# MAGIC-AI4Med/KEEP

Measured on AMD Instinct MI355X. Metric: 224x224 tiles encoded/sec (whole node), higher is better.
Workload: dtype fp16+mxfp4

## Files before the change

### keep_amd/csrc/common.h

```cpp
#pragma once
#include <hip/hip_runtime.h>
#include <stdint.h>

typedef _Float16 f16;
typedef _Float16 f16x2 __attribute__((ext_vector_type(2)));
typedef _Float16 f16x4 __attribute__((ext_vector_type(4)));
typedef _Float16 f16x8 __attribute__((ext_vector_type(8)));
typedef float f32x4 __attribute__((ext_vector_type(4)));
typedef float f32x16 __attribute__((ext_vector_type(16)));

#define KEEP_WAVE 64

__device__ __forceinline__ void split_f16(float x, f16& hi, f16& lo) {
    asm("" : "+v"(x));
    hi = (f16)x;
    lo = (f16)(x - (float)hi);
}

__device__ __forceinline__ unsigned char clip8_fixed(int v) {
    v >>= 22;
    return (unsigned char)(v < 0 ? 0 : (v > 255 ? 255 : v));
}
__device__ __forceinline__ float gelu_erf(float x) {
    return 0.5f * x * (1.0f + erff(x * 0.70710678118654752440f));
}

__device__ __forceinline__ float wave_sum(float v) {
#pragma unroll
    for (int o = 32; o > 0; o >>= 1) v += __shfl_xor(v, o);
    return v;
}
__device__ __forceinline__ float wave_max(float v) {
#pragma unroll
    for (int o = 32; o > 0; o >>= 1) v = fmaxf(v, __shfl_xor(v, o));
    return v;
}

__host__ __device__ __forceinline__ int64_t blk_off(int m, int k, int KT) {
    return ((int64_t)(m >> 8) * KT + (k >> 5)) * 8192 + ((m & 255) << 5) + (k & 31);
}
static inline size_t blk_elems(int64_t M, int64_t K) { return (size_t)((M + 255) / 256 * 256) * (size_t)K; }


struct KeepTune {
    int gemm_impl = 0;
    int gemm_skinny_m = 320;
    int skinny_wide = 1;
    int gemm_splitk_tiles = 64;
    int sgemv_m = 16;
    int ln_impl = 2;
    int attn_waves = 16;
    int gemm_persistent = 1;
    int gemm_ablate = 0;
    long long* dbg = nullptr;
};

enum GemmEpi : int {
    EPI_F16      = 0,
    EPI_GELU_F16 = 1,
    EPI_RESID_LS = 2,
    EPI_PATCH    = 3,
    EPI_RESID_F32= 4,
    EPI_PARTIAL  = 5,
    EPI_TOP2     = 6,
};

struct GemmParams {
    const f16* a_hi; const f16* a_lo;
    const f16* w_hi; const f16* w_lo;
    int M, N, K;
    int nseg;
    int comp;
    const unsigned char* a_q; const unsigned char* a_sc;
    const unsigned char* w_q; const unsigned char* w_sc;
    unsigned char* out_q; unsigned char* out_sc;
    const float* bias;
    const float* ls;
    const float* pos;
    float* resid;
    float* out_f32;
    f16* out_hi; f16* out_lo;
    int out_kt;
    int patches_per_img;
    const float* ln_gamma; const float* ln_beta; float ln_eps;
    f16* ln_out_hi; f16* ln_out_lo; float* ln_out_f32;
    int top2_c; float* top2_partial; int top2_kpad;
    int impl_hint;
    int ksplit;
    float* splitk_ws; size_t splitk_bytes;
    long long* dbg;
    int ablate;
    const KeepTune* tune;
};

int launch_gemm_f16(const GemmParams& p, int epi, hipStream_t s);
constexpr int GEMM_DID_LN = 1;
constexpr int SKINNY_MAX_M = 1024;
constexpr size_t SKINNY_WS_BYTES = (size_t)448 * 256 * 256 * 4;
int launch_gemm_splitk_reduce(const GemmParams& p, int epi, const float* ws, int S, hipStream_t s);
int launch_gemm_f16_skinny(const GemmParams& p, int epi, float* ws, size_t ws_bytes, hipStream_t s);

struct AttnParams {
    const f16* qkv_hi; const f16* qkv_lo;
    f16* out_hi; f16* out_lo;
    int out_kt;
    const int64_t* mask;
    int batch, ntok, heads;
    int q_rows;
    int split;
    f16* cls_hi; f16* cls_lo;
    float* part_ws; size_t part_bytes;
    int key0, kcount;
    float* part_out; const float* part_in;
    float scale;
    long long* dbg;
    const KeepTune* tune;
};
int launch_attention(const AttnParams& p, hipStream_t s);
int launch_attention_long(const AttnParams& p, hipStream_t s);
constexpr int ATT_PART_FLOATS = 66;
int launch_attention_cls_probs(const f16* qkv_hi, const f16* qkv_lo, int batch, int ntok, int heads, float scale, float* out, hipStream_t s);
constexpr int ROLLOUT_MAX_TOKENS = 272;
int launch_attention_rollout_step(const f16* qkv_hi, const f16* qkv_lo, int batch, int ntok, int heads, float scale, float residual,
                                  const float* r_in, float* r_out, int q_rows, float* a_tmp, hipStream_t s);

struct LnParams {
    const float* x; int64_t x_stride;
    const float* add;
    const float* gamma; const float* beta;
    int rows, D; float eps;
    f16* out_hi; f16* out_lo;
    int out_kt;
    float* out_f32; int64_t out_f32_stride;
    unsigned char* out_q; unsigned char* out_sc;
    int out_q_hi_only;
    const KeepTune* tune;
};
int launch_layernorm(const LnParams& p, hipStream_t s);

enum SgemmAct : int { ACT_NONE = 0, ACT_GELU = 1, ACT_TANH = 2 };
struct SgemmParams {
    const float* a; int64_t lda;
    const float* b; int64_t ldb;
    float* out; int64_t ldo;
    const float* bias;
    int M, N, K;
    float scale; int act;
    const KeepTune* tune;
};
int launch_sgemm_f32(const SgemmParams& p, hipStream_t s);

__device__ __forceinline__ int block_exclusive_scan256(int v, int* s, int* total) {
    const int t = threadIdx.x;
    s[t] = v;
    __syncthreads();
    for (int o = 1; o < 256; o <<= 1) {
        const int a = t >= o ? s[t - o] : 0;
        __syncthreads();
        s[t] += a;
        __syncthreads();
    }
    const int incl = s[t];
    *total = s[255];
    __syncthreads();
    return incl - v;
}

void launch_region_grid(const unsigned char* region, int64_t row_stride, int ps, int gx, int64_t ncells, int patch, int step, int sat_min,
                        int min_pixels, unsigned char* keep, int* counts, int* offsets, int32_t* cell_xy, int64_t* n_out, hipStream_t s);
void launch_region_check_cells(const int32_t* cell_xy, int B, int64_t H, int64_t W, int patch, int* bad, hipStream_t s);
void launch_region_patches_u8(const unsigned char* region, int64_t row_stride, int ps, const int32_t* cell_xy, int B, int patch,
                              const int* xb, const int* xk, int xks, const int* yb, const int* yk, int yks, unsigned char* tmp,
                              unsigned char* out, hipStream_t s);
void launch_region_compact(const unsigned char* keep, int gx, int64_t ncells, int step, int* counts, int* offsets, int32_t* cell_xy,
                           int64_t* n_out, hipStream_t s);
constexpr int REGION_MAX_PATCH = 32768;
constexpr int REGION_GRID_CHUNK = 2048;

constexpr int64_t TISSUE_MAX_PIXELS = (int64_t)1 << 30;
int launch_tissue_median_hist(const unsigned char* thumb, int64_t row_stride, int ps, int h, int w, int ksize, unsigned char* med, int* hist,
                              hipStream_t s);
void launch_tissue_mask(const unsigned char* med, int h, int w, int thr, int close, int min_hole, int min_area, unsigned char* tmp, int* labels,
                        int* info, int* err, unsigned char* mask, hipStream_t s);
void launch_tissue_grid_cells(const unsigned char* mask, int64_t mh, int64_t mw, int64_t ds, int gx, int64_t ncells, int patch, int step,
                              int64_t ox, int64_t oy, int mode, unsigned char* keep, hipStream_t s);

void launch_cc_label(const unsigned char* img, int h, int w, int conn8, int* labels, int* info, int* err, hipStream_t s);

constexpr int REGIONS_COLS = 14;
constexpr int REGIONS_SCAN_CHUNK = 2048;
void launch_regions_label(const unsigned char* mask, int h, int w, int conn8, int min_area, int* roots, int* info, int* counts, int* offsets,
                          int* err, int* labels_out, int64_t* n_out, hipStream_t s);
void launch_regions_table(const int* labels, int h, int w, int64_t n, const int64_t* acc, int64_t* table, hipStream_t s);

constexpr int64_t OUTLINE_MAX_PIXELS = (int64_t)1 << 28;
constexpr int OUTLINE_COLS = 8;
constexpr int OUTLINE_CHUNK = 2048;
constexpr int OUTLINE_FLAG_WORDS = 96;
constexpr int OUTLINE_MAX_WIDTH = 16;
size_t outline_count_workspace_bytes(int64_t npix);
// ... 114 lines not shown
```

### keep_amd/csrc/engine.hip

```cpp
#include "handle.h"
#include "quant4.h"

#include <algorithm>
#include <cmath>
#include <cstring>

namespace {

constexpr int64_t TXT_GRAPH_ROWS = 4096;

const char* kTagNames[T_COUNT] = {
    "vit.im2col", "vit.patch", "vit.ln", "vit.qkv", "vit.attn", "vit.proj", "vit.fc1", "vit.fc2", "vit.head",
    "text.embed", "text.ln", "text.qkv", "text.attn", "text.out", "text.ffn1", "text.ffn2", "text.pool", "sim",
    "vit.qkv.x", "vit.attn.x", "vit.proj.x", "vit.fc1.x", "vit.fc2.x", "vit.tail"};

struct Scope {
    keep_handle* h; int tag; hipStream_t s;
    Scope(keep_handle* h_, int t, hipStream_t s_) : h(h_), tag(t), s(s_) { h->prof_begin(tag, s); }
    ~Scope() { h->prof_end(tag, s); }
};

size_t align_up(size_t x, size_t a = 256) { return (x + a - 1) / a * a; }

struct Carver {
// ... 501 lines not shown

struct RollArgs { int start; float residual; float* out; char* scratch; int64_t scratch_bytes; };
struct RollPlan { size_t buf, lane, total; };
RollPlan rollout_scratch(int64_t B, int ntok, const VitPlan& plan) {
    RollPlan r{};
    const int64_t live = std::min<int64_t>(B, plan.per * plan.lanes);
    r.buf = align_up((size_t)plan.per * ntok * ntok * sizeof(float));
    r.lane = 3 * r.buf;
    r.total = r.lane * (size_t)((live + plan.per - 1) / plan.per);
    return r;
}
int encode_image_run(keep_handle* h, const void* pixels, int pix_dtype, int64_t B, float* out, hipStream_t s, int gh = 14, int gw = 14,
                     int tap_block = -1, float* tap_out = nullptr, const RollArgs* roll = nullptr) {
    const int ntok = gh * gw + 1;
    const bool g14 = gh == 14 && gw == 14;
    const float* pos = nullptr;
    int rc = vit_pos_table(h, gh, gw, &pos);
    if (rc) return rc;
    const size_t px = pix_dtype == KEEP_PIX_F32 ? 4 : (pix_dtype == KEEP_PIX_U8_HWC ? 1 : 2);
    const size_t tile_vals = (size_t)3 * (gh * 16) * (gw * 16);
    const bool graph = h->use_graphs && !h->prof_mode && B * ntok <= SKINNY_MAX_M && B <= h->max_tiles && !tap_out && !roll;
    const VitPlan plan = vit_plan(h, B, ntok, tile_vals * px, graph);
    const RollPlan rp = roll ? rollout_scratch(B, ntok, plan) : RollPlan{};
    if (roll && (int64_t)rp.total > roll->scratch_bytes)
        return h->fail(KEEP_EINVAL, "rollout scratch of %lld bytes, %lld needed (keep_rollout_scratch_bytes)", (long long)roll->scratch_bytes, (long long)rp.total);
    rc = ensure_arena(h, plan.total);
    if (rc) return rc;
    if (graph) {
        const size_t ob = (size_t)B * h->proj_dim * sizeof(float);
        char* st_pix = h->arena + plan.o_pix;
        float* st_out = (float*)(h->arena + plan.o_out);
        HIPCHK(h, hipMemcpyAsync(st_pix, pixels, (size_t)B * tile_vals * px, hipMemcpyDeviceToDevice, s));
        char key[96];
        if (g14) snprintf(key, sizeof key, "img|%lld|%d|%d", (long long)B, pix_dtype, h->precision);
        else snprintf(key, sizeof key, "img|%lld|%d|%d|%dx%d", (long long)B, pix_dtype, h->precision, gh, gw);
        rc = graph_run(h, key, s, [&](hipStream_t cs) {
            VitLane L{};
            L.Bc = (int)B; L.pixels = st_pix; L.pix_dtype = pix_dtype; L.out = st_out; L.s = cs;
            L.gh = gh; L.gw = gw; L.ntok = ntok; L.pos = pos;
            L.ws = carve_vit(h, h->arena, L.Bc, plan.split, ntok);
            int r = vit_begin(h, L);
            for (int i = 0; !r && i < h->vit_depth; ++i) r = vit_layer(h, L, i);
            return r ? r : vit_end(h, L);
        });
        if (rc) return rc;
        HIPCHK(h, hipMemcpyAsync(out, st_out, ob, hipMemcpyDeviceToDevice, s));
        return KEEP_OK;
    }
    const int lanes = plan.lanes;
    const int64_t per = plan.per;
    if (lanes > 1) {
        if (!h->ev_fork) HIPCHK(h, hipEventCreateWithFlags(&h->ev_fork, hipEventDisableTiming));
        for (int l = 0; l < lanes; ++l) {
            if (!h->aux[l]) HIPCHK(h, hipStreamCreateWithFlags(&h->aux[l], hipStreamNonBlocking));
            if (!h->ev_join[l]) HIPCHK(h, hipEventCreateWithFlags(&h->ev_join[l], hipEventDisableTiming));
        }
        HIPCHK(h, hipEventRecord(h->ev_fork, s));
        for (int l = 0; l < lanes; ++l) HIPCHK(h, hipStreamWaitEvent(h->aux[l], h->ev_fork, 0));
    }
    for (int64_t b0 = 0; b0 < B; b0 += per * lanes) {
        VitLane L[4];
        int nl = 0;
        for (int l = 0; l < lanes; ++l) {
            const int64_t lo = b0 + l * per;
            if (lo >= B) break;
            VitLane& x = L[nl++];
            x.Bc = (int)((B - lo) < per ? (B - lo) : per);
            x.pixels = (const char*)pixels + (size_t)lo * tile_vals * px;
            x.pix_dtype = pix_dtype;
            x.out = out + lo * h->proj_dim;
            x.s = lanes > 1 ? h->aux[l] : s;
            x.gh = gh; x.gw = gw; x.ntok = ntok; x.pos = pos;
            if (tap_out) { x.tap_block = tap_block; x.tap_out = tap_out + lo * h->vit_heads * ntok; }
            if (roll) {
                float* base = (float*)(roll->scratch + (size_t)l * rp.lane);
                x.roll_start = roll->start; x.roll_res = roll->residual; x.roll_out = roll->out + lo * ntok;
                x.roll_r[0] = base; x.roll_r[1] = base + rp.buf / sizeof(float); x.roll_a = base + 2 * (rp.buf / sizeof(float));
            }
            x.ws = carve_vit(h, h->arena + (size_t)l * plan.lane_bytes, x.Bc, plan.split, ntok);
        }
        for (int l = 0; l < nl; ++l) if ((rc = vit_begin(h, L[l]))) return rc;
        for (int i = 0; i < h->vit_depth; ++i)
            for (int l = 0; l < nl; ++l) if ((rc = vit_layer(h, L[l], i))) return rc;
        for (int l = 0; l < nl; ++l) if ((rc = vit_end(h, L[l]))) return rc;
    }
    if (lanes > 1)
        for (int l = 0; l < lanes; ++l) {
            HIPCHK(h, hipEventRecord(h->ev_join[l], h->aux[l]));
            HIPCHK(h, hipStreamWaitEvent(s, h->ev_join[l], 0));
        }
    return KEEP_OK;
}


int similarity_run(keep_handle* h, const float* img, const float* txt, int64_t N, int64_t P, int64_t D, float scale, int mode,
                   void* out, int32_t* argmax_out, hipStream_t s) {
    Scope sc(h, T_SIM, s);
    if (h->tune.sgemv_m > 0 && launch_sim_small(img, txt, (int)N, (int)P, (int)D, scale, mode, out, argmax_out, s) == 0)
        return check_launch(h, "similarity");
    if (h->tune.sgemv_m > 0 && launch_sim_mid(img, txt, (int)N, (int)P, (int)D, scale, mode, out, argmax_out, s) == 0)
        return check_launch(h, "similarity");
    float* logits = (float*)out;
    const bool need_tmp = (mode == KEEP_SIM_ARGMAX && !out) || mode == KEEP_SIM_SOFTMAX_F16 || mode == KEEP_SIM_TOP2SCORE;
    const int nb = (int)((N + 255) / 256);
    if (need_tmp) {
        const size_t bytes = align_up((size_t)N * P * 4) + align_up((size_t)nb * 4) + 256;
        int rc = ensure_arena(h, bytes);
        if (rc) return rc;
        logits = (float*)h->arena;
    }
    SgemmParams g{};
    g.tune = &h->tune;
    g.a = img; g.lda = D; g.b = txt; g.ldb = D; g.out = logits; g.ldo = P; g.bias = nullptr;
    g.M = (int)N; g.N = (int)P; g.K = (int)D; g.act = ACT_NONE;
    g.scale = (mode == KEEP_SIM_RAW || mode == KEEP_SIM_ARGMAX) ? scale : 1.0f;
    if (launch_sgemm_f32(g, s)) return h->fail(KEEP_EUNSUPPORTED, "similarity shape");
    if (mode == KEEP_SIM_ARGMAX) launch_row_argmax(logits, (int)N, (int)P, argmax_out, s);
    else if (mode == KEEP_SIM_SOFTMAX) launch_row_softmax(logits, (int)N, (int)P, scale, logits, s);
    else if (mode == KEEP_SIM_SOFTMAX_F16) launch_row_softmax_f16(logits, (int)N, (int)P, scale, (f16*)out, s);
    else if (mode == KEEP_SIM_TOP2SCORE) {
        float* partial = (float*)(h->arena + align_up((size_t)N * P * 4));
        launch_top2_score(logits, (int)N, (int)P, partial, (float*)out, s);
    }
    return check_launch(h, "similarity");
}


enum : unsigned { OPT_REPLAN = 1,
                  OPT_WRITEONLY = 2 };
struct Opt { const char* name; int keep_handle::* hm; int KeepTune::* tm; bool is_bool; int lo, hi; const char* msg; unsigned flags; };
constexpr int NO_MAX = 0x7fffffff;
static_assert(SKINNY_MAX_M == 1024, "the gemm_skinny_m message below spells the bound out");
const Opt kOptions[] = {
    {"graphs", &keep_handle::use_graphs, nullptr, true, 0, 0, nullptr, 0},
    {"strict_blocks", &keep_handle::strict_blocks, nullptr, false, 0, NO_MAX, "strict_blocks < 0", 0},
    {"comp_full_blocks", &keep_handle::comp_full_blocks, nullptr, false, 0, NO_MAX, "comp_full_blocks < 0", OPT_REPLAN},
    {"comp_mlp_blocks", &keep_handle::comp_mlp_blocks, nullptr, false, 0, NO_MAX, "comp_mlp_blocks < 0", OPT_REPLAN},
    {"comp_qkv", &keep_handle::comp_qkv, nullptr, true, 0, 0, nullptr, OPT_REPLAN},
    {"comp_qkv_from", &keep_handle::comp_qkv_from, nullptr, false, 0, NO_MAX, "comp_qkv_from < 0", OPT_REPLAN},
    {"comp_min_tiles", &keep_handle::comp_min_tiles, nullptr, false, 24, NO_MAX, "comp_min_tiles must be >= 24 (the compensated product needs the 256x256 kernel)", 0},
    {"fused_screening", &keep_handle::fused_screening, nullptr, false, 0, 2, "fused_screening must be 0..2", OPT_WRITEONLY},
    {"max_tiles", &keep_handle::max_tiles, nullptr, false, 1, NO_MAX, "max_tiles < 1", 0},
    {"max_prompts", &keep_handle::max_prompts, nullptr, false, 1, NO_MAX, "max_prompts < 1", 0},
    {"cls_tail", &keep_handle::cls_tail, nullptr, true, 0, 0, nullptr, 0},
    {"patch_split", &keep_handle::patch_split, nullptr, true, 0, 0, nullptr, 0},
    {"grid_plan", &keep_handle::grid_plan, nullptr, false, 0, 2, "grid_plan must be 0, 1 or 2", 0},
    {"bias_correction", &keep_handle::bias_correction, nullptr, true, 0, 0, nullptr, 0},
    {"streams", &keep_handle::n_streams, nullptr, false, 1, 4, "streams must be 1..4", 0},
    {"lane_min_tiles", &keep_handle::lane_min_tiles, nullptr, false, 6, NO_MAX, "lane_min_tiles must be >= 6", OPT_WRITEONLY},
    {"gemm_persistent", nullptr, &KeepTune::gemm_persistent, false, 0, 1024, "gemm_persistent must be 0..1024", 0},
    {"gemm_splitk_tiles", nullptr, &KeepTune::gemm_splitk_tiles, false, 0, 256, "gemm_splitk_tiles must be 0..256", 0},
    {"sgemv_m", nullptr, &KeepTune::sgemv_m, false, 0, 16, "sgemv_m must be 0..16", 0},
    {"skinny_wide", nullptr, &KeepTune::skinny_wide, true, 0, 0, nullptr, 0},
    {"gemm_skinny_m", nullptr, &KeepTune::gemm_skinny_m, false, 0, SKINNY_MAX_M, "gemm_skinny_m must be 0..1024", 0},
    {"ln_impl", nullptr, &KeepTune::ln_impl, false, 0, 2, "ln_impl must be 0, 1 or 2", 0},
};
const Opt* find_opt(const char* name) {
    for (const Opt& o : kOptions) if (!strcmp(name, o.name)) return &o;
    return nullptr;
}
int& opt_value(keep_handle* h, const Opt& o) { return o.hm ? h->*o.hm : h->tune.*o.tm; }

}

extern "C" {

const char* keep_version(void) { return "keep_hip 0.1 (gfx950)"; }

int keep_create(int device_id, keep_handle** out) {
    if (!out) return KEEP_EINVAL;
    *out = nullptr;
    int n = 0;
    if (hipGetDeviceCount(&n) != hipSuccess || device_id < 0 || device_id >= n) return KEEP_EHIP;
    DevGuard guard(device_id);
    if (!guard.ok) return KEEP_EHIP;
    keep_handle* h = new keep_handle();
    h->device = device_id;
    if (hipMalloc(&h->err_flag, 4 * sizeof(int)) != hipSuccess) { delete h; return KEEP_ENOMEM; }
    hipMemset(h->err_flag, 0, 4 * sizeof(int));
    *out = h;
    return KEEP_OK;
}

int keep_destroy(keep_handle* h) {
    if (!h) return KEEP_OK;
    DevGuard guard(h->device);
    hipDeviceSynchronize();
    h->prof_collect();
    for (auto& e : h->pool) { hipEventDestroy(e.first); hipEventDestroy(e.second); }
    for (auto& kv : h->w) { if (kv.second.f32) hipFree(kv.second.f32); if (kv.second.hi) hipFree(kv.second.hi); if (kv.second.lo) hipFree(kv.second.lo);
                            if (kv.second.q) hipFree(kv.second.q); if (kv.second.sc) hipFree(kv.second.sc); }
    if (h->tune.dbg) hipFree(h->tune.dbg);
    for (float* v : h->owned_vecs) hipFree(v);
    h->free_cal();
    h->drop_pos_cache();
    for (auto& l : h->blayers) { if (l.qkv.hi) hipFree(l.qkv.hi); if (l.qkv.lo) hipFree(l.qkv.lo); if (l.qkv_b) hipFree(l.qkv_b); }
    drop_graphs(h);
    if (h->cap_stream) hipStreamDestroy(h->cap_stream);
    if (h->arena) hipFree(h->arena);
    if (h->cls_buf) hipFree(h->cls_buf);
    if (h->err_flag) hipFree(h->err_flag);
    for (int l = 0; l < 4; ++l) { if (h->aux[l]) hipStreamDestroy(h->aux[l]); if (h->ev_join[l]) hipEventDestroy(h->ev_join[l]); }
    if (h->ev_fork) hipEventDestroy(h->ev_fork);
    delete h;
    return KEEP_OK;
}

const char* keep_last_error(keep_handle* h) { return h ? h->err.c_str() : "null handle"; }

int keep_set_option(keep_handle* h, const char* name, double value) {
    if (!h || !name) return KEEP_EINVAL;
    const std::string n(name);
    const int v = (int)value;
    ++h->opt_epoch;
    KeepTune& t = h->tune;
    if (const Opt* o = find_opt(name)) {
        if (!o->is_bool && (v < o->lo || v > o->hi)) return h->fail(KEEP_EINVAL, "%s", o->msg);
        opt_value(h, *o) = o->is_bool ? (v ? 1 : 0) : v;
        if (o->flags & OPT_REPLAN) h->plan_from_prefix();
        if (o->hm == &keep_handle::cls_tail && h->bias_ready && h->cal_cls_tail != h->cls_tail) h->bias_ready = false;
    }
    else if (n == "label_margin") { if (!(value >= 0.0) || value > 2.0) return h->fail(KEEP_EINVAL, "label_margin must be in [0, 2]"); h->label_margin = (float)value; }
    else if (n == "precision") { if (v != KEEP_PREC_FP16 && v != KEEP_PREC_STRICT && v != KEEP_PREC_COMP) return h->fail(KEEP_EINVAL, "precision %d", v); h->precision = v; }
    else if (n == "proj_impl") { if (v != 0 && v != 2128) return h->fail(KEEP_EINVAL, "proj_impl must be 0 or 2128"); h->proj_impl = v; }
    else if (n == "attn_waves") { if (v != 4 && v != 8 && v != 16) return h->fail(KEEP_EINVAL, "attn_waves must be 4, 8 or 16 (16: persistent double-buffered kernel for the image tower)"); t.attn_waves = v; }
    else if (n == "gemm_impl") { if (v != 0 && v != 128 && v != 256) return h->fail(KEEP_EINVAL, "gemm_impl %d (0, 128, 256)", v); t.gemm_impl = v; }
#ifdef KEEP_DIAGNOSTICS
    else if (n == "gemm_ablate") { t.gemm_ablate = v; }
    else if (n == "gemm_dbg") {
        if (v && !t.dbg) { HIPCHK(h, hipMalloc(&t.dbg, (size_t)65536 * 4 * sizeof(long long))); HIPCHK(h, hipMemset(t.dbg, 0, (size_t)65536 * 4 * sizeof(long long))); }
        if (!v && t.dbg) { hipFree(t.dbg); t.dbg = nullptr; }
    }
#endif
    else return h->fail(KEEP_EINVAL, "unknown option %s", name);
    return KEEP_OK;
}
double keep_get_option(keep_handle* h, const char* name) {
    if (!h || !name) return -1;
    const std::string n(name);
    if (const Opt* o = find_opt(name)) return (o->flags & OPT_WRITEONLY) ? -1 : opt_value(h, *o);
    if (n == "label_margin") return h->label_margin;
    if (n == "precision") return h->precision;
    if (n == "proj_impl") return h->proj_impl;
    if (n == "attn_waves") return h->tune.attn_waves;
    if (n == "gemm_impl") return h->tune.gemm_impl;
    if (n == "plan_custom") return h->plan_custom ? 1 : 0;
    if (n == "bias_ready") return h->bias_ready ? 1 : 0;
    if (n == "graph_count") return (double)h->graphs.size();
    return -1;
}

int keep_set_block_precision(keep_handle* h, int block, int attn_mode, int mlp_mode) {
    if (!h) return KEEP_EINVAL;
    if (block < 0 || block >= keep_handle::MAX_BLOCKS) return h->fail(KEEP_EINVAL, "block %d outside 0..%d", block, keep_handle::MAX_BLOCKS - 1);
    if (attn_mode > KEEP_ATTN_COMPQKV_PROJ_CLS || mlp_mode > KEEP_MLP_CLS) return h->fail(KEEP_EINVAL, "attn_mode %d (0..5) / mlp_mode %d (0..4); negative = leave", attn_mode, mlp_mode);
    ++h->opt_epoch;
    if (attn_mode >= 0) h->attn_mode[block] = (unsigned char)attn_mode;
    if (mlp_mode >= 0) h->mlp_mode[block] = (unsigned char)mlp_mode;
    h->plan_custom = true;
    return KEEP_OK;
}
int keep_get_block_precision(keep_handle* h, int block, int* attn_mode, int* mlp_mode) {
    if (!h) return KEEP_EINVAL;
    if (block < 0 || block >= keep_handle::MAX_BLOCKS) return h->fail(KEEP_EINVAL, "block %d outside 0..%d", block, keep_handle::MAX_BLOCKS - 1);
    if (attn_mode) *attn_mode = h->attn_mode[block];
    if (mlp_mode) *mlp_mode = h->mlp_mode[block];
    return KEEP_OK;
}

int keep_reserve(keep_handle* h, int64_t tiles, int64_t prompts, int64_t seq) {
    if (!h || !h->finalized) return h ? h->fail(KEEP_ESTATE, "weights not finalised") : KEEP_EINVAL;
    KEEP_ON_DEVICE(h);
    size_t need = 0;
    if (tiles > 0 && h->vit_depth) need = vit_plan(h, tiles, 197, (size_t)3 * 224 * 224 * 4, tiles * 197 <= SKINNY_MAX_M).total;
    if (prompts > 0 && seq > 0 && h->bert_layers) need = std::max(need, txt_plan(h, prompts, seq, prompts * seq <= TXT_GRAPH_ROWS).total);
    return ensure_arena(h, need);
}
int64_t keep_workspace_bytes(keep_handle* h) { return h ? (int64_t)h->arena_bytes : 0; }

int keep_encode_image(keep_handle* h, const void* pixels, int pix_dtype, int64_t B, float* out, void* stream) {
    if (!h) return KEEP_EINVAL;
    if (!h->finalized || !h->vit_depth) return h->fail(KEEP_ESTATE, "image tower not loaded / finalised");
    if (!pixels || !out || B < 0) return h->fail(KEEP_EINVAL, "null pointer or negative batch");
    if (pix_dtype < KEEP_PIX_F32 || pix_dtype > KEEP_PIX_U8_HWC) return h->fail(KEEP_EINVAL, "pixel dtype %d", pix_dtype);
    if (B == 0) return KEEP_OK;
    KEEP_ON_DEVICE(h);
    return encode_image_run(h, pixels, pix_dtype, B, out, (hipStream_t)stream);
}

int keep_encode_image_hw(keep_handle* h, const void* pixels, int pix_dtype, int64_t B, int64_t H, int64_t W, float* out, void* stream) {
    if (!h) return KEEP_EINVAL;
    if (!h->finalized || !h->vit_depth) return h->fail(KEEP_ESTATE, "image tower not loaded / finalised");
    if (!pixels || !out || B < 0) return h->fail(KEEP_EINVAL, "null pointer or negative batch");
    if (pix_dtype < KEEP_PIX_F32 || pix_dtype > KEEP_PIX_U8_HWC) return h->fail(KEEP_EINVAL, "pixel dtype %d", pix_dtype);
    if (H < 16 || W < 16 || H % 16 || W % 16) return h->fail(KEEP_EINVAL, "image size %lldx%lld: H and W must be positive multiples of 16", (long long)H, (long long)W);
    const int64_t gh = H / 16, gw = W / 16;
    if (gh * gw + 1 > 65536) return h->fail(KEEP_EUNSUPPORTED, "image size %lldx%lld: more than 65536 patches", (long long)H, (long long)W);
    if (B == 0) return KEEP_OK;
    KEEP_ON_DEVICE(h);
    const int prec = h->precision;
    if (!(gh == 14 && gw == 14) && !h->grid_keeps_plan((int)(gh * gw + 1)) && prec == KEEP_PREC_COMP) h->precision = KEEP_PREC_STRICT;
    const int rc = encode_image_run(h, pixels, pix_dtype, B, out, (hipStream_t)stream, (int)gh, (int)gw);
    h->precision = prec;
    return rc;
}

// ... 451 lines not shown
```

### keep_amd/csrc/gemm_f16_skinny.hip

```cpp
#include "gemm_epilogue.h"

namespace keepk {

constexpr int SK_BM = 32, SK_BN = 128;

__global__ __launch_bounds__(256)
void gemm_skinny_partial_kernel(GemmParams p, float* __restrict__ part, int steps_per_split) {
    const int lane = threadIdx.x & 63, wave = threadIdx.x >> 6;
    const int n0 = blockIdx.x * SK_BN + wave * 32, m0 = blockIdx.y * SK_BM, split = blockIdx.z;
    const int KT = p.K / 32;
    const int kt0 = split * steps_per_split;
    const int kt1 = min(KT, kt0 + steps_per_split);
    const int r = lane & 31, half = lane >> 5;
    const int m = m0 + r, n = n0 + r;
    const int64_t a_base = (int64_t)(m >> 8) * KT * 8192 + ((m & 255) << 5) + half * 8;
    const int64_t w_base = (int64_t)(n >> 8) * KT * 8192 + ((n & 255) << 5) + half * 8;
    f32x16 acc;
#pragma unroll
    for (int i = 0; i < 16; ++i) acc[i] = 0.f;
    for (int seg = 0; seg < p.nseg; ++seg) {
        const f16* A = (seg == 1 ? p.a_lo : p.a_hi) + a_base;
        const f16* W = (seg == 2 ? p.w_lo : p.w_hi) + w_base;
        int kt = kt0;
        for (; kt + 2 <= kt1; kt += 2) {
            const f16x8 a0 = *reinterpret_cast<const f16x8*>(A + (int64_t)kt * 8192);
            const f16x8 w0 = *reinterpret_cast<const f16x8*>(W + (int64_t)kt * 8192);
            const f16x8 a1 = *reinterpret_cast<const f16x8*>(A + (int64_t)kt * 8192 + 16);
            const f16x8 w1 = *reinterpret_cast<const f16x8*>(W + (int64_t)kt * 8192 + 16);
            const f16x8 a2 = *reinterpret_cast<const f16x8*>(A + (int64_t)(kt + 1) * 8192);
            const f16x8 w2 = *reinterpret_cast<const f16x8*>(W + (int64_t)(kt + 1) * 8192);
            const f16x8 a3 = *reinterpret_cast<const f16x8*>(A + (int64_t)(kt + 1) * 8192 + 16);
            const f16x8 w3 = *reinterpret_cast<const f16x8*>(W + (int64_t)(kt + 1) * 8192 + 16);
            acc = __builtin_amdgcn_mfma_f32_32x32x16_f16(w0, a0, acc, 0, 0, 0);
            acc = __builtin_amdgcn_mfma_f32_32x32x16_f16(w1, a1, acc, 0, 0, 0);
            acc = __builtin_amdgcn_mfma_f32_32x32x16_f16(w2, a2, acc, 0, 0, 0);
            acc = __builtin_amdgcn_mfma_f32_32x32x16_f16(w3, a3, acc, 0, 0, 0);
        }
        for (; kt < kt1; ++kt) {
            const f16x8 a0 = *reinterpret_cast<const f16x8*>(A + (int64_t)kt * 8192);
            const f16x8 w0 = *reinterpret_cast<const f16x8*>(W + (int64_t)kt * 8192);
            const f16x8 a1 = *reinterpret_cast<const f16x8*>(A + (int64_t)kt * 8192 + 16);
            const f16x8 w1 = *reinterpret_cast<const f16x8*>(W + (int64_t)kt * 8192 + 16);
            acc = __builtin_amdgcn_mfma_f32_32x32x16_f16(w0, a0, acc, 0, 0, 0);
            acc = __builtin_amdgcn_mfma_f32_32x32x16_f16(w1, a1, acc, 0, 0, 0);
        }
    }
    if (m < p.M) {
        float* o = part + ((int64_t)split * p.M + m) * p.N + n0 + half * 4;
#pragma unroll
        for (int rg = 0; rg < 4; ++rg) {
            f32x4 v;
#pragma unroll
            for (int e = 0; e < 4; ++e) v[e] = acc[rg * 4 + e];
            *reinterpret_cast<f32x4*>(o + rg * 8) = v;
        }
    }
}

constexpr int SK2_BM = 128, SK2_BN = 128;

__global__ __launch_bounds__(256)
void gemm_skinny_partial_wide_kernel(GemmParams p, float* __restrict__ part, int steps_per_split) {
    const int lane = threadIdx.x & 63, wave = threadIdx.x >> 6;
    const int wm = wave >> 1, wn = wave & 1;
    const int n0 = blockIdx.x * SK2_BN + wn * 64, m0 = blockIdx.y * SK2_BM + wm * 64, split = blockIdx.z;
    const int KT = p.K / 32;
    const int kt0 = split * steps_per_split;
    const int kt1 = min(KT, kt0 + steps_per_split);
    const int r = lane & 31, half = lane >> 5;
    int64_t a_base[2], w_base[2];
#pragma unroll
    for (int f = 0; f < 2; ++f) {
        const int m = m0 + f * 32 + r, n = n0 + f * 32 + r;
        a_base[f] = (int64_t)(m >> 8) * KT * 8192 + ((m & 255) << 5) + half * 8;
        w_base[f] = (int64_t)(n >> 8) * KT * 8192 + ((n & 255) << 5) + half * 8;
    }
    f32x16 acc[2][2];
#pragma unroll
    for (int i = 0; i < 2; ++i)
#pragma unroll
        for (int j = 0; j < 2; ++j)
#pragma unroll
            for (int e = 0; e < 16; ++e) acc[i][j][e] = 0.f;
    const int nk = kt1 - kt0, steps = nk > 0 ? nk * p.nseg : 0;
    auto frag = [&](int st, f16x8 (&a)[2][2], f16x8 (&w)[2][2]) {
        const int seg = st / nk, kt = kt0 + (st - seg * nk);
        const f16* A = seg == 1 ? p.a_lo : p.a_hi;
        const f16* W = seg == 2 ? p.w_lo : p.w_hi;
#pragma unroll
        for (int f = 0; f < 2; ++f)
#pragma unroll
            for (int k = 0; k < 2; ++k) {
                a[f][k] = *reinterpret_cast<const f16x8*>(A + a_base[f] + (int64_t)kt * 8192 + k * 16);
                w[f][k] = *reinterpret_cast<const f16x8*>(W + w_base[f] + (int64_t)kt * 8192 + k * 16);
            }
    };
    auto fma8 = [&](const f16x8 (&a)[2][2], const f16x8 (&w)[2][2]) {
#pragma unroll
        for (int k = 0; k < 2; ++k)
#pragma unroll
            for (int i = 0; i < 2; ++i)
#pragma unroll
                for (int j = 0; j < 2; ++j) acc[i][j] = __builtin_amdgcn_mfma_f32_32x32x16_f16(w[j][k], a[i][k], acc[i][j], 0, 0, 0);
    };
    f16x8 a0[2][2], w0[2][2], a1[2][2], w1[2][2];
    if (steps > 0) frag(0, a0, w0);
    int st = 0;
    for (; st + 2 <= steps; st += 2) {
        frag(st + 1, a1, w1);
        fma8(a0, w0);
        if (st + 2 < steps) frag(st + 2, a0, w0);
        fma8(a1, w1);
    }
    if (st < steps) fma8(a0, w0);
#pragma unroll
    for (int i = 0; i < 2; ++i) {
        const int m = m0 + i * 32 + r;
        if (m >= p.M) continue;
#pragma unroll
        for (int j = 0; j < 2; ++j) {
            float* o = part + ((int64_t)split * p.M + m) * p.N + n0 + j * 32 + half * 4;
#pragma unroll
            for (int rg = 0; rg < 4; ++rg) {
                f32x4 v;
#pragma unroll
                for (int e = 0; e < 4; ++e) v[e] = acc[i][j][rg * 4 + e];
                *reinterpret_cast<f32x4*>(o + rg * 8) = v;
            }
        }
    }
}

template <int EPI>
__global__ __launch_bounds__(256)
void gemm_skinny_reduce_kernel(GemmParams p, const float* __restrict__ part, int S) {
    const int64_t idx = (int64_t)blockIdx.x * 256 + threadIdx.x;
    const int nq = p.N / 4;
    if (idx >= (int64_t)p.M * nq) return;
    const int m = (int)(idx / nq), n = (int)(idx - (int64_t)m * nq) * 4;
    f32x4 v = *reinterpret_cast<const f32x4*>(part + (int64_t)m * p.N + n);
    for (int s = 1; s < S; ++s) {
        const f32x4 x = *reinterpret_cast<const f32x4*>(part + ((int64_t)s * p.M + m) * p.N + n);
#pragma unroll
        for (int e = 0; e < 4; ++e) v[e] += x[e];
    }
    const f32x4 bias = *reinterpret_cast<const f32x4*>(p.bias + n);
#pragma unroll
    for (int e = 0; e < 4; ++e) v[e] += bias[e];
    int prow; int64_t orow;
    gemm_epilogue_row<EPI>(p, m, prow, orow);
    const int64_t o = orow * p.N + n;
    if (EPI == EPI_F16 || EPI == EPI_GELU_F16) {
        if (EPI == EPI_GELU_F16) {
            f32x2 a = {v[0], v[1]}, b = {v[2], v[3]};
            if (p.out_lo) { a = gelu_fast2(a); b = gelu_fast2(b); }
            else { a = gelu_fast2_fp16(a); b = gelu_fast2_fp16(b); }
            v[0] = a[0]; v[1] = a[1]; v[2] = b[0]; v[3] = b[1];
        }
        f16x4 h, l;
#pragma unroll
        for (int e = 0; e < 4; ++e) { f16 hh, ll; split_f16(v[e], hh, ll); h[e] = hh; l[e] = ll; }
        const int64_t oo = p.out_kt > 0 ? blk_off((int)orow, n, p.out_kt) : o;
        *reinterpret_cast<f16x4*>(p.out_hi + oo) = h;
        if (p.out_lo) *reinterpret_cast<f16x4*>(p.out_lo + oo) = l;
    } else if (EPI == EPI_RESID_LS) {
        const f32x4 g = *reinterpret_cast<const f32x4*>(p.ls + n);
        f32x4 r = *reinterpret_cast<const f32x4*>(p.resid + o);
#pragma unroll
        for (int e = 0; e < 4; ++e) r[e] += __fmul_rn(g[e], v[e]);
        *reinterpret_cast<f32x4*>(p.resid + o) = r;
    } else if (EPI == EPI_PATCH) {
        const f32x4 pe = *reinterpret_cast<const f32x4*>(p.pos + (int64_t)prow * p.N + n);
#pragma unroll
        for (int e = 0; e < 4; ++e) v[e] += pe[e];
        *reinterpret_cast<f32x4*>(p.resid + o) = v;
    } else {
        const f32x4 r = *reinterpret_cast<const f32x4*>(p.resid + o);
#pragma unroll
        for (int e = 0; e < 4; ++e) v[e] += r[e];
        *reinterpret_cast<f32x4*>(p.out_f32 + o) = v;
    }
}

template <int EPI>
__global__ __launch_bounds__(256)
void gemm_skinny_reduce_ln_kernel(GemmParams p, const float* __restrict__ part, int S) {
    __shared__ float red[2][4];
    const int m = blockIdx.x, t = threadIdx.x, n = t * 4;
    const bool on = n < p.N;
    f32x4 r = {0.f, 0.f, 0.f, 0.f};
    if (on) {
        f32x4 v = *reinterpret_cast<const f32x4*>(part + (int64_t)m * p.N + n);
        for (int s = 1; s < S; ++s) {
            const f32x4 x = *reinterpret_cast<const f32x4*>(part + ((int64_t)s * p.M + m) * p.N + n);
#pragma unroll
            for (int e = 0; e < 4; ++e) v[e] += x[e];
        }
        const f32x4 bias = *reinterpret_cast<const f32x4*>(p.bias + n);
        const int64_t o = (int64_t)m * p.N + n;
        r = *reinterpret_cast<const f32x4*>(p.resid + o);
        if (EPI == EPI_RESID_LS) {
            const f32x4 g = *reinterpret_cast<const f32x4*>(p.ls + n);
#pragma unroll
            for (int e = 0; e < 4; ++e) r[e] += __fmul_rn(g[e], v[e] + bias[e]);
            *reinterpret_cast<f32x4*>(p.resid + o) = r;
        } else {
#pragma unroll
            for (int e = 0; e < 4; ++e) r[e] = (v[e] + bias[e]) + r[e];
            if (p.ln_out_f32 != p.out_f32) *reinterpret_cast<f32x4*>(p.out_f32 + o) = r;
        }
    }
    const int wave = t >> 6, lane = t & 63;
    float sum = wave_sum(r[0] + r[1] + r[2] + r[3]);
    if (lane == 0) red[0][wave] = sum;
    __syncthreads();
    const float mean = (red[0][0] + red[0][1] + red[0][2] + red[0][3]) / (float)p.N;
    float sq = 0.f;
    if (on) {
#pragma unroll
        for (int e = 0; e < 4; ++e) { r[e] -= mean; sq += r[e] * r[e]; }
    }
    sq = wave_sum(sq);
    if (lane == 0) red[1][wave] = sq;
    __syncthreads();
    const float rstd = 1.0f / sqrtf((red[1][0] + red[1][1] + red[1][2] + red[1][3]) / (float)p.N + p.ln_eps);
    if (!on) return;
    const f32x4 g = *reinterpret_cast<const f32x4*>(p.ln_gamma + n);
    const f32x4 bt = *reinterpret_cast<const f32x4*>(p.ln_beta + n);
    f32x4 y; f16x4 h, l;
#pragma unroll
    for (int e = 0; e < 4; ++e) {
        y[e] = r[e] * rstd * g[e] + bt[e];
        f16 hh, ll; split_f16(y[e], hh, ll); h[e] = hh; l[e] = ll;
    }
    if (p.ln_out_f32) *reinterpret_cast<f32x4*>(p.ln_out_f32 + (int64_t)m * p.N + n) = y;
    const int64_t oo = blk_off(m, n, p.N / 32);
    *reinterpret_cast<f16x4*>(p.ln_out_hi + oo) = h;
    if (p.ln_out_lo) *reinterpret_cast<f16x4*>(p.ln_out_lo + oo) = l;
}

}
using namespace keepk;

bool skinny_wide(int M, const KeepTune* t = nullptr) { return M >= 64 && (!t || t->skinny_wide); }

int skinny_splits(int M, int N, int K, const KeepTune* t = nullptr) {
    const bool wide = skinny_wide(M, t);
    const int tiles = wide ? ((M + SK2_BM - 1) / SK2_BM) * (N / SK2_BN) : ((M + SK_BM - 1) / SK_BM) * (N / SK_BN), ks = K / 32;
    int S = ((wide ? 256 : 768) + tiles - 1) / tiles;
    if (S > ks / 2) S = ks / 2;
    if (S > 16) S = 16;
    return S < 1 ? 1 : S;
}

size_t skinny_ws_bytes(int M, int N, int K) { return (size_t)skinny_splits(M, N, K) * M * N * sizeof(float); }

int launch_gemm_f16_skinny(const GemmParams& p, int epi, float* ws, size_t ws_bytes, hipStream_t s) {
    if (!ws || p.N % SK_BN || p.K % 32 || p.M < 1) return -1;
    const int S = skinny_splits(p.M, p.N, p.K, p.tune);
    if ((size_t)S * p.M * p.N * sizeof(float) > ws_bytes) return -1;
    const int KT = p.K / 32, per = (KT + S - 1) / S;
    dim3 block(256);
    if (skinny_wide(p.M, p.tune)) hipLaunchKernelGGL(gemm_skinny_partial_wide_kernel, dim3(p.N / SK2_BN, (p.M + SK2_BM - 1) / SK2_BM, S), block, 0, s, p, ws, per);
    else hipLaunchKernelGGL(gemm_skinny_partial_kernel, dim3(p.N / SK_BN, (p.M + SK_BM - 1) / SK_BM, S), block, 0, s, p, ws, per);
    return launch_gemm_splitk_reduce(p, epi, ws, S, s);
}

int launch_gemm_splitk_reduce(const GemmParams& p, int epi, const float* ws, int S, hipStream_t s) {
    dim3 block(256);
    if (p.ln_gamma && p.ln_out_hi && (epi == EPI_RESID_LS || epi == EPI_RESID_F32) && p.N <= 1024) {
        if (epi == EPI_RESID_LS) hipLaunchKernelGGL(gemm_skinny_reduce_ln_kernel<EPI_RESID_LS>, dim3(p.M), block, 0, s, p, ws, S);
        else hipLaunchKernelGGL(gemm_skinny_reduce_ln_kernel<EPI_RESID_F32>, dim3(p.M), block, 0, s, p, ws, S);
        return GEMM_DID_LN;
    }
    const int64_t items = (int64_t)p.M * (p.N / 4);
    dim3 rg((unsigned)((items + 255) / 256));
    switch (epi) {
        case EPI_F16:       hipLaunchKernelGGL(gemm_skinny_reduce_kernel<EPI_F16>, rg, block, 0, s, p, ws, S); break;
        case EPI_GELU_F16:  hipLaunchKernelGGL(gemm_skinny_reduce_kernel<EPI_GELU_F16>, rg, block, 0, s, p, ws, S); break;
        case EPI_RESID_LS:  hipLaunchKernelGGL(gemm_skinny_reduce_kernel<EPI_RESID_LS>, rg, block, 0, s, p, ws, S); break;
        case EPI_PATCH:     hipLaunchKernelGGL(gemm_skinny_reduce_kernel<EPI_PATCH>, rg, block, 0, s, p, ws, S); break;
        default:            hipLaunchKernelGGL(gemm_skinny_reduce_kernel<EPI_RESID_F32>, rg, block, 0, s, p, ws, S); break;
    }
    return 0;
}
```

Before: 7043.

## Add fused three-segment skinny wide GEMM kernel with register ring prefetch

Adds a split-K skinny wide kernel for compensated (hi/lo, nseg==3) products that handles all three product segments in one pass over K. It loads A and W hi/lo slices together and keeps separate main and correction accumulators. The older kernel loops over segments and re-streams the operands three times. A DEPTH-slot register ring prefetches upcoming K slices to hide global-load latency. The cost is much higher register pressure (two 4x4 accumulator sets plus four slices of four planes), which may reduce occupancy or cause spills.

```diff
diff --git a/keep_amd/csrc/common.h b/keep_amd/csrc/common.h
--- a/keep_amd/csrc/common.h
+++ b/keep_amd/csrc/common.h
@@ -46,6 +46,7 @@
     int gemm_impl = 0;
     int gemm_skinny_m = 320;
     int skinny_wide = 1;
+    int skinny_fused = 1;
     int gemm_splitk_tiles = 64;
     int sgemv_m = 16;
     int ln_impl = 2;
diff --git a/keep_amd/csrc/engine.hip b/keep_amd/csrc/engine.hip
--- a/keep_amd/csrc/engine.hip
+++ b/keep_amd/csrc/engine.hip
@@ -677,6 +677,7 @@
     {"gemm_splitk_tiles", nullptr, &KeepTune::gemm_splitk_tiles, false, 0, 256, "gemm_splitk_tiles must be 0..256", 0},
     {"sgemv_m", nullptr, &KeepTune::sgemv_m, false, 0, 16, "sgemv_m must be 0..16", 0},
     {"skinny_wide", nullptr, &KeepTune::skinny_wide, true, 0, 0, nullptr, 0},
+    {"skinny_fused", nullptr, &KeepTune::skinny_fused, true, 0, 0, nullptr, 0},
     {"gemm_skinny_m", nullptr, &KeepTune::gemm_skinny_m, false, 0, SKINNY_MAX_M, "gemm_skinny_m must be 0..1024", 0},
     {"ln_impl", nullptr, &KeepTune::ln_impl, false, 0, 2, "ln_impl must be 0, 1 or 2", 0},
 };
diff --git a/keep_amd/csrc/gemm_f16_skinny.hip b/keep_amd/csrc/gemm_f16_skinny.hip
--- a/keep_amd/csrc/gemm_f16_skinny.hip
+++ b/keep_amd/csrc/gemm_f16_skinny.hip
@@ -131,6 +131,101 @@
     }
 }
 
+#ifndef SK2_FUSED_DEPTH
+#define SK2_FUSED_DEPTH 4
+#endif
+
+struct Sk2Slice { f16x8 ah[4], al[4], wh[4], wl[4]; };
+struct Sk2Planes { const f16* ah; const f16* al; const f16* wh; const f16* wl; int64_t a[4], w[4]; };
+
+__device__ __forceinline__ void sk2_load(Sk2Slice& s, const Sk2Planes& q, int kt) {
+#pragma unroll
+    for (int f = 0; f < 4; ++f) {
+        const int64_t ao = q.a[f] + (int64_t)kt * 8192, wo = q.w[f] + (int64_t)kt * 8192;
+        s.ah[f] = *reinterpret_cast<const f16x8*>(q.ah + ao);
+        s.al[f] = *reinterpret_cast<const f16x8*>(q.al + ao);
+        s.wh[f] = *reinterpret_cast<const f16x8*>(q.wh + wo);
+        s.wl[f] = *reinterpret_cast<const f16x8*>(q.wl + wo);
+    }
+}
+
+__device__ __forceinline__ void sk2_fma48(const Sk2Slice& s, f32x4 (&main)[4][4], f32x4 (&corr)[4][4]) {
+#pragma unroll
+    for (int i = 0; i < 4; ++i)
+#pragma unroll
+        for (int j = 0; j < 4; ++j) main[i][j] = __builtin_amdgcn_mfma_f32_16x16x32_f16(s.wh[j], s.ah[i], main[i][j], 0, 0, 0);
+#pragma unroll
+    for (int i = 0; i < 4; ++i)
+#pragma unroll
+        for (int j = 0; j < 4; ++j) corr[i][j] = __builtin_amdgcn_mfma_f32_16x16x32_f16(s.wh[j], s.al[i], corr[i][j], 0, 0, 0);
+#pragma unroll
+    for (int i = 0; i < 4; ++i)
+#pragma unroll
+        for (int j = 0; j < 4; ++j) corr[i][j] = __builtin_amdgcn_mfma_f32_16x16x32_f16(s.wl[j], s.ah[i], corr[i][j], 0, 0, 0);
+}
+
+template <int DEPTH>
+__global__ __launch_bounds__(256)
+void gemm_skinny_partial_wide_fused_kernel(GemmParams p, float* __restrict__ part, int steps_per_split) {
+    const int lane = threadIdx.x & 63, wave = threadIdx.x >> 6;
+    const int wm = wave >> 1, wn = wave & 1;
+    const int n0 = blockIdx.x * SK2_BN + wn * 64, m0 = blockIdx.y * SK2_BM + wm * 64, split = blockIdx.z;
+    const int KT = p.K / 32;
+    const int kt0 = split * steps_per_split;
+    const int kt1 = min(KT, kt0 + steps_per_split);
+    const int r = lane & 15, quarter = lane >> 4;
+    Sk2Planes q{p.a_hi, p.a_lo, p.w_hi, p.w_lo, {0, 0, 0, 0}, {0, 0, 0, 0}};
+#pragma unroll
+    for (int f = 0; f < 4; ++f) {
+        const int m = m0 + f * 16 + r, n = n0 + f * 16 + r;
+        q.a[f] = (int64_t)(m >> 8) * KT * 8192 + ((m & 255) << 5) + quarter * 8;
+        q.w[f] = (int64_t)(n >> 8) * KT * 8192 + ((n & 255) << 5) + quarter * 8;
+    }
+    f32x4 main[4][4], corr[4][4];
+#pragma unroll
+    for (int i = 0; i < 4; ++i)
+#pragma unroll
+        for (int j = 0; j < 4; ++j)
+#pragma unroll
+            for (int e = 0; e < 4; ++e) main[i][j][e] = corr[i][j][e] = 0.f;
+    Sk2Slice ring[DEPTH];
+    const int nk = kt1 - kt0 > 0 ? kt1 - kt0 : 0;
+    const int head = nk % DEPTH;
+#pragma unroll
+    for (int i = 0; i < DEPTH - 1; ++i)
+        if (i < head) sk2_load(ring[i], q, kt0 + i);
+#pragma unroll
+    for (int i = 0; i < DEPTH - 1; ++i)
+        if (i < head) sk2_fma48(ring[i], main, corr);
+    int kt = kt0 + head;
+    if (kt < kt1) {
+#pragma unroll
+        for (int i = 0; i < DEPTH; ++i) sk2_load(ring[i], q, kt + i);
+        for (; kt + 2 * DEPTH <= kt1; kt += DEPTH) {
+#pragma unroll
+            for (int i = 0; i < DEPTH; ++i) {
+                sk2_fma48(ring[i], main, corr);
+                sk2_load(ring[i], q, kt + DEPTH + i);
+            }
+        }
+#pragma unroll
+        for (int i = 0; i < DEPTH; ++i) sk2_fma48(ring[i], main, corr);
+    }
+#pragma unroll
+    for (int i = 0; i < 4; ++i) {
+        const int m = m0 + i * 16 + r;
+        if (m >= p.M) continue;
+        float* o = part + ((int64_t)split * p.M + m) * p.N + n0 + quarter * 4;
+#pragma unroll
+        for (int j = 0; j < 4; ++j) {
+            f32x4 v;
+#pragma unroll
+            for (int e = 0; e < 4; ++e) v[e] = main[i][j][e] + corr[i][j][e];
+            *reinterpret_cast<f32x4*>(o + j * 16) = v;
+        }
+    }
+}
+
 template <int EPI>
 __global__ __launch_bounds__(256)
 void gemm_skinny_reduce_kernel(GemmParams p, const float* __restrict__ part, int S) {
@@ -244,6 +339,8 @@
 
 bool skinny_wide(int M, const KeepTune* t = nullptr) { return M >= 64 && (!t || t->skinny_wide); }
 
+bool skinny_fused(int M, int nseg, const KeepTune* t = nullptr) { return nseg == 3 && skinny_wide(M, t) && (!t || t->skinny_fused); }
+
 int skinny_splits(int M, int N, int K, const KeepTune* t = nullptr) {
     const bool wide = skinny_wide(M, t);
     const int tiles = wide ? ((M + SK2_BM - 1) / SK2_BM) * (N / SK2_BN) : ((M + SK_BM - 1) / SK_BM) * (N / SK_BN), ks = K / 32;
@@ -261,7 +358,8 @@
     if ((size_t)S * p.M * p.N * sizeof(float) > ws_bytes) return -1;
     const int KT = p.K / 32, per = (KT + S - 1) / S;
     dim3 block(256);
-    if (skinny_wide(p.M, p.tune)) hipLaunchKernelGGL(gemm_skinny_partial_wide_kernel, dim3(p.N / SK2_BN, (p.M + SK2_BM - 1) / SK2_BM, S), block, 0, s, p, ws, per);
+    if (skinny_fused(p.M, p.nseg, p.tune)) hipLaunchKernelGGL(gemm_skinny_partial_wide_fused_kernel<SK2_FUSED_DEPTH>, dim3(p.N / SK2_BN, (p.M + SK2_BM - 1) / SK2_BM, S), block, 0, s, p, ws, per);
+    else if (skinny_wide(p.M, p.tune)) hipLaunchKernelGGL(gemm_skinny_partial_wide_kernel, dim3(p.N / SK2_BN, (p.M + SK2_BM - 1) / SK2_BM, S), block, 0, s, p, ws, per);
     else hipLaunchKernelGGL(gemm_skinny_partial_kernel, dim3(p.N / SK_BN, (p.M + SK_BM - 1) / SK_BM, S), block, 0, s, p, ws, per);
     return launch_gemm_splitk_reduce(p, epi, ws, S, s);
 }
```

Measured after the change: 7048 (median of 2 runs). About the same (+0.1%).
